# tomtor/HDL-deflate

Measured on AMD Instinct MI355X. Metric: compress_input_throughput (CWINDOW=32, MATCH10=True, static tree), higher is better.
Workload: dtype u8; 1 GPU; BASELINE configs[1]: 1048576 x 2048 B blocks, families 1-4 (test_deflate.py:38-66), distinct blocks, HBM-resident; cwindow=32, maxmatch=10, blocks_per_gpu=1048576, block_bytes=2048

## Files before the change

hdl_deflate_amd/csrc/hdlz_compress.hip:

```cpp
#include <hip/hip_runtime.h>
#include <stdint.h>
#include "hdlz_device.h"
#include "hdlz_compress_common.h"

namespace hdlz {

#ifndef HDLZ_HP_SEARCH
#define HDLZ_HP_SEARCH 1
#define HDLZ_HP_EXTEND 0
#define HDLZ_HP_REST 0
#endif
#ifdef HDLZ_TILE_TIMING
#define TT_DECL() uint32_t tacc[13] = {0, 0, 0, 0, 0, 0, 0, 0, 0, 0, 0, 0, 0}, tlast = (uint32_t)__builtin_readcyclecounter(); \
        const uint32_t tt_c0 = tlast, tt_r0 = (uint32_t)__builtin_amdgcn_s_memrealtime()
#define TT(k) do { const uint32_t t_ = (uint32_t)__builtin_readcyclecounter(); tacc[k] += t_ - tlast; tlast = t_; } while (0)
#define TT_TILE() tacc[12] += 1u
#else
#define TT_DECL() do {} while (0)
#define TT(k) do {} while (0)
#define TT_TILE() do {} while (0)
#endif

__device__ __forceinline__ void store_words(uint32_t* __restrict__ dst, const uint32_t* lsrc, uint32_t words, uint32_t lane) {
    const uint32_t nq = words >> 2;
    for (uint32_t q0 = 0; q0 < nq; q0 += 64u) {
        const uint32_t q = q0 + lane;
        if (q < nq) {
            const v4 v = *reinterpret_cast<const v4*>(lsrc + 4u * q);
            asm volatile("global_store_dwordx4 %0, %1, off\n\ts_nop 1" :: "v"(dst + 4u * q), "v"(v) : "memory");
        }
    }
    if (lane < (words & 3u)) dst[4u * nq + lane] = lsrc[4u * nq + lane];
}

template <int NCH, bool FULLWIN, bool ONE_TILE, bool ENDBITS = false>
__global__ __launch_bounds__(64) __attribute__((amdgpu_waves_per_eu(waves_eu<NCH>(), waves_eu<NCH>()))) void k_compress(CompressArgs a) {
    constexpr bool HASH = wide_hash<NCH>();
    constexpr bool BITS = ONE_TILE && NCH == 1 && search_bits();
    __shared__ typename std::conditional<HASH, WaveLdsNoOut, typename std::conditional<BITS, WaveLdsBits, WaveLds>::type>::type lds;
    __shared__ typename std::conditional<HASH, HashLds<NCH>, uint32_t>::type hl;
    uint32_t* const lout = lds_out(lds, hl);
    const uint32_t lane = threadIdx.x;

    if constexpr (!BITS) {
        fill_luts<NCH>(lds.lut, lane);
        __syncthreads();
    }

    const uint32_t cw4 = 4u * (uint32_t)a.cwindow;
    const uint32_t kmax = (uint32_t)a.maxmatch;
    uint8_t* lin8 = reinterpret_cast<uint8_t*>(lds.in);
    const uint8_t* lut8 = reinterpret_cast<const uint8_t*>(lds.lut);
    uint8_t* out8 = reinterpret_cast<uint8_t*>(lout);

    const uint32_t fixed_st = a.in_len < 5u ? (uint32_t)HDLZ_E_SHORT_INPUT
                            : (ONE_TILE && a.in_len > (uint32_t)TILE) ? (uint32_t)HDLZ_E_BAD_PARAM
                            : (uint64_t)out_bound(a.in_len) > a.out_pitch ? (uint32_t)HDLZ_E_OUT_CAPACITY : (uint32_t)HDLZ_OK;
    auto block_params = [&](uint64_t blk, const uint8_t*& src, uint32_t& n) -> uint32_t {
        if (!a.in_off) {
            src = a.in + blk * a.in_pitch;
            n = a.in_len;
            return fixed_st;
        }
        const uint64_t off = a.in_off[blk];
        const uint64_t len64 = a.in_off[blk + 1] - off;
        if (len64 >= 0x80000000ull) return HDLZ_E_BAD_PARAM;
        n = (uint32_t)len64;
        src = a.in + off;
        if (n < 5u) return HDLZ_E_SHORT_INPUT;
        if (ONE_TILE && n > (uint32_t)TILE) return HDLZ_E_BAD_PARAM;
        if ((uint64_t)out_bound(n) > a.out_pitch) return HDLZ_E_OUT_CAPACITY;
        return HDLZ_OK;
    };
    constexpr uint32_t NCHUNK = (TILE + LOOKAHEAD) / 16;
    const uint32_t in_base = (uint32_t)__builtin_amdgcn_readfirstlane((int)(uint32_t)reinterpret_cast<uintptr_t>(lin8)) + (uint32_t)HALO;
    auto request_tile = [&](const uint8_t* tsrc, uint32_t nfull) {
        if (lane < nfull) lds_dma16(tsrc + 16u * lane, in_base);
        if (lane + 64u < nfull) lds_dma16(tsrc + 16u * (lane + 64u), in_base + 1024u);
        if (nfull > 128u) { if (lane == 0u) lds_dma16(tsrc + 2048u, in_base + 2048u); }
    };
    [[maybe_unused]] const uint32_t lut_base = (uint32_t)__builtin_amdgcn_readfirstlane((int)(uint32_t)reinterpret_cast<uintptr_t>(lds.lut));
    auto request_lut = [&]() {
        const uint8_t* t = reinterpret_cast<const uint8_t*>(FIXED_LUT.e) + 16u * lane;
        lds_dma16(t, lut_base);
        lds_dma16(t + 1024u, lut_base + 1024u);
    };

#if defined(HDLZ_STRIDE_PLAIN) || defined(HDLZ_TILE_TIMING)
    constexpr bool MOVING_COLUMN = false;
#else
    constexpr bool MOVING_COLUMN = BITS;
#endif
    [[maybe_unused]] uint64_t row0 = 0;
    [[maybe_unused]] uint32_t col = blockIdx.x;
    auto next_block = [&](uint64_t& blk) {
        if constexpr (MOVING_COLUMN) {
            row0 += gridDim.x;
            col = col + 1u == gridDim.x ? 0u : col + 1u;
            blk = row0 + col;
        } else blk += gridDim.x;
    };
    TT_DECL();
    for (uint64_t blk = blockIdx.x; blk < a.nblocks; next_block(blk)) {
        const uint8_t* src;
        uint32_t n;
        const uint32_t bst = block_params(blk, src, n);
        if (bst != HDLZ_OK) {
            if (lane == 0) {
                a.out_len[blk] = 0; a.status[blk] = bst;
                if constexpr (ENDBITS) a.end_bits[blk] = 0;
            }
            continue;
        }
        uint32_t* __restrict__ outw = reinterpret_cast<uint32_t*>(a.out + blk * a.out_pitch);
        const uint32_t mis = (uint32_t)(reinterpret_cast<uintptr_t>(src) & 3u);
        const bool aligned16 = (reinterpret_cast<uintptr_t>(src) & 15u) == 0;

        uint32_t gw = 0;
        uint32_t base_bits = HEADER_BITS;
        uint32_t carry_word = HEADER_WORD;
        uint32_t skip_in = 0;
        uint32_t ad_a = 0, ad_w = 0;
        uint32_t wm = (n - min(lane * (uint32_t)RUN, n)) % ADLER_MOD;

        for (uint32_t t0 = 0; t0 < n; t0 += TILE) {
            if (blk == blockIdx.x) TT(10); else TT(0);
            HDLZ_MARK("stage");
            const uint32_t nfull = min((n - t0) >> 4, NCHUNK);
            wave_lds_order();
            lds.in[lane] = t0 != 0 ? lds.in[(TILE / 4) + lane] : 0u;
            asm volatile("s_waitcnt lgkmcnt(0)" ::: "memory");
            request_tile(src + t0, nfull);
            {
                const uint32_t part = (nfull < NCHUNK && ((n - t0) & 15u) != 0u) ? 1u : 0u;
                for (uint32_t c = nfull + part + lane; c < NCHUNK; c += 64) *reinterpret_cast<uint4*>(lin8 + HALO + c * 16u) = make_uint4(0, 0, 0, 0);
                if (part) {
                    if (lane == 0u) *reinterpret_cast<uint4*>(lin8 + HALO + nfull * 16u) = load_chunk16(src, t0 + nfull * 16u, n, aligned16, mis);
                }
            }
            if constexpr (!HASH && !BITS) zero_bit_buffer(lout, lane, carry_word);
            asm volatile("s_waitcnt vmcnt(0)" ::: "memory");
            wave_lds_order();

            const uint32_t run_dw = (HALO / 4) + lane * (RUN / 4);
            const uint32_t p_run = t0 + lane * RUN;
            const uint32_t nrem = n - min(p_run, n);
            uint32_t best[RUN], tok[RUN], code[RUN];
            [[maybe_unused]] uint32_t oww[12];
            [[maybe_unused]] bool any = true;
            [[maybe_unused]] uint32_t planes[7];
            if constexpr (BITS) {
                load_own(lds.in, run_dw, oww);
                asm volatile("s_waitcnt lgkmcnt(0)" ::: "memory");
                wave_lds_order();
            }
            TT(1);
            if constexpr (!HASH) __builtin_amdgcn_s_setprio(0);
            else __builtin_amdgcn_s_setprio(HDLZ_HP_SEARCH);
            HDLZ_MARK("search");
            if constexpr (HASH) {
                match_search_hash<NCH>(lds.in, hl, lane, (uint32_t)a.cwindow, best);
                zero_bit_buffer(lout, lane, carry_word);
            }
#ifndef HDLZ_SEARCH_KEYS
            else if constexpr (BITS)
                any = match_search_bits<true>(oww[0], oww[1], oww[2], oww[3], oww[4], oww[5], oww[6], oww[7], planes, lds.neq + lane, end_cap_word((int32_t)(n - t0) - 2, lane * (uint32_t)RUN));
#endif
            else match_search<NCH, ONE_TILE && NCH == 1>(lds.in, run_dw, best);
            {
                TT(2);
                HDLZ_MARK("adler");
                uint32_t ow[12];
                if constexpr (BITS) {
#pragma unroll
                    for (int k = 0; k < 12; k++) ow[k] = oww[k];
                } else load_own(lds.in, run_dw, ow);
                {
                    uint32_t sa, sc;
                    adler_run(ow, sa, sc);
                    ad_a += sa;
                    ad_w = (ad_w + __umul24(wm, sa) + (4u * ADLER_MOD - sc)) % ADLER_MOD;
                    wm = wm >= (uint32_t)(TILE % ADLER_MOD) ? wm - (uint32_t)(TILE % ADLER_MOD) : wm + (ADLER_MOD - (uint32_t)(TILE % ADLER_MOD));
                    if (((t0 >> 11) & 0x3FFFFu) == 0x3FFFFu) ad_a %= ADLER_MOD;
                    asm volatile("" : "+v"(ad_a), "+v"(ad_w), "+v"(wm));
                }
                TT(3);
                if constexpr (!HASH) __builtin_amdgcn_s_setprio(1);
                else __builtin_amdgcn_s_setprio(HDLZ_HP_EXTEND);
                HDLZ_MARK("extend");
                if constexpr (BITS) {
                    if (any) {
#if HDLZ_EXT_SDWA
                        uint32_t Q[8];
                        search_result_packed(planes, Q);
                        wave_lds_order();
                        make_tokens_bits_packed<FULLWIN>(lds.neq, lane, ow, Q, cw4, kmax, tok, (int32_t)(n - t0));
#else
                        search_result_bytes(planes, best);
                        wave_lds_order();
                        make_tokens_bits<FULLWIN>(lds.neq, lane, ow, best, cw4, kmax, 4u * min(p_run, 32u * NCH), tok, (int32_t)(n - t0));
#endif
                    } else {
                        literal_tokens(ow, tok);
                        asm volatile("s_waitcnt lgkmcnt(0)" ::: "memory");
                        wave_lds_order();
                    }
                } else
                make_tokens<NCH, FULLWIN, true>(lds.in, HALO + lane * RUN, ow, best, cw4, kmax, 4u * min(p_run, 32u * NCH), nrem, tok, (int32_t)(n - t0));
            }
            pin(tok);
            PHASE_FENCE();
            TT(4);
            if constexpr (BITS) {
                HDLZ_MARK("zero");
                wave_lds_order();
                request_lut();
                zero_bit_buffer(lout, lane, carry_word);
            }
            if constexpr (HASH) __builtin_amdgcn_s_setprio(HDLZ_HP_REST);
            HDLZ_MARK("parse");
            uint32_t myskip = 0;
            if (!BITS || any) {
                const uint64_t P = run_transfer(tok);
                TT(5);
                HDLZ_MARK("chain");
                myskip = chain_skips(P, lane, skip_in);
            }
            pin(tok); asm volatile("" : "+v"(myskip));
            PHASE_FENCE();
            TT(6);
            HDLZ_MARK("codes");
            if constexpr (BITS) {
                asm volatile("s_waitcnt vmcnt(0)" ::: "memory");
                wave_lds_order();
            }
            uint32_t lane_bits = token_codes<NCH, false>(lut8, tok, myskip, 0u, code);
            pin(code);
            PHASE_FENCE();
            TT(7);
            HDLZ_MARK("scan");
            uint32_t incl = wave_scan_incl(lane_bits);
            const uint32_t tile_bits_all = (uint32_t)__builtin_amdgcn_readlane((int)incl, 63);
            pin(code); asm volatile("" : "+v"(incl), "+v"(lane_bits));
            PHASE_FENCE();
            TT(8);
            HDLZ_MARK("scatter");
            scatter_codes(out8, code, base_bits + incl - lane_bits);
            TT(9);
            HDLZ_MARK("flush");
            wave_lds_order();
            TT(10);

            const bool last = ONE_TILE || (t0 + TILE >= n);
            if (!last) {
                const uint32_t end_bits = base_bits + tile_bits_all;
                const uint32_t full = end_bits >> 5;
                store_words(outw + gw, lout, full, lane);
                carry_word = lout[full];
                gw += full;
                base_bits = end_bits & 31u;
            } else {
                const uint32_t ninv = t0 + TILE - n;
                const uint32_t end_bits = base_bits + tile_bits_all - PAD_BITS * ninv;
                if (lane < 4u) wipe_behind(lout, end_bits, lane);
                uint32_t s1, s2;
                adler_finish(wave_sum(ad_a % ADLER_MOD), wave_sum(ad_w), n, s1, s2);
                const uint32_t nbytes = block_nbytes(end_bits);
                wave_lds_order();
                if (lane == 0) put_adler(out8, nbytes, s1, s2);
                wave_lds_order();
                const uint32_t total = nbytes + 4u;
                const uint32_t words = (total + 3u) >> 2;
                store_words(outw + gw, lout, words, lane);
                if (lane == 0) {
                    a.out_len[blk] = gw * 4u + total;
                    a.status[blk] = HDLZ_OK;
                    if constexpr (ENDBITS) a.end_bits[blk] = 32ull * gw + end_bits;
                }
            }
            TT(11);
            TT_TILE();
        }
    }
#ifdef HDLZ_TILE_TIMING
    asm volatile("s_waitcnt vmcnt(0)" ::: "memory");
    if (lane == 0) {
        uint64_t blk = blockIdx.x;
#pragma unroll
        for (int k = 0; k < 13; k++, blk += gridDim.x)
            if (blk < a.nblocks) { a.out_len[blk] = tacc[k]; a.status[blk] = 0u; }
        if (blk < a.nblocks) { a.out_len[blk] = (uint32_t)__builtin_readcyclecounter() - tt_c0; a.status[blk] = 0u; }
        blk += gridDim.x;
        if (blk < a.nblocks) { a.out_len[blk] = (uint32_t)__builtin_amdgcn_s_memrealtime() - tt_r0; a.status[blk] = 0u; }
    }
#endif
}

template __global__ void k_compress<1, true, true>(CompressArgs);
template __global__ void k_compress<1, false, true>(CompressArgs);
template __global__ void k_compress<1, true, false>(CompressArgs);
template __global__ void k_compress<1, false, false>(CompressArgs);
template __global__ void k_compress<2, true, false>(CompressArgs);
template __global__ void k_compress<2, false, false>(CompressArgs);
template __global__ void k_compress<8, true, false>(CompressArgs);
template __global__ void k_compress<8, false, false>(CompressArgs);
template __global__ void k_compress<1, true, true, true>(CompressArgs);
template __global__ void k_compress<1, false, true, true>(CompressArgs);
template __global__ void k_compress<1, true, false, true>(CompressArgs);
template __global__ void k_compress<1, false, false, true>(CompressArgs);
template __global__ void k_compress<2, true, false, true>(CompressArgs);
template __global__ void k_compress<2, false, false, true>(CompressArgs);
template __global__ void k_compress<8, true, false, true>(CompressArgs);
template __global__ void k_compress<8, false, false, true>(CompressArgs);

hipError_t launch_compress(const CompressArgs& a, hipStream_t stream) {
    if (a.nblocks == 0) return hipSuccess;
    static int ncu_of[64] = {0};
    int dev = 0;
    if (hipGetDevice(&dev) != hipSuccess) return hipGetLastError();
    int ncu = (dev >= 0 && dev < 64) ? ncu_of[dev] : 0;
    if (ncu == 0) {
        if (hipDeviceGetAttribute(&ncu, hipDeviceAttributeMultiprocessorCount, dev) != hipSuccess) return hipGetLastError();
        if (ncu <= 0) ncu = 256;
        if (dev >= 0 && dev < 64) ncu_of[dev] = ncu;
    }
    if (!a.end_bits && a.in_len >= 5u && a.in_len <= 1024u && a.out_pitch >= (uint64_t)out_bound(a.in_len) &&
        (a.in_off || ((a.in_pitch & 15u) == 0 && (reinterpret_cast<uintptr_t>(a.in) & 15u) == 0)))
        return launch_compress_small(a, stream, ncu);
    uint64_t g = (uint64_t)ncu * 256u;
    if (g > a.nblocks) g = a.nblocks;
    const dim3 grid((unsigned)g), block(64);
    const bool one_tile = a.in_len >= 5u && a.in_len <= (uint32_t)TILE;
    with_window(a.cwindow, [&](auto N, auto FW) {
        constexpr int NCH = decltype(N)::value;
        constexpr bool FULLWIN = decltype(FW)::value;
        if (a.end_bits) {
            if (NCH == 1 && one_tile) hipLaunchKernelGGL((k_compress<1, FULLWIN, true, true>), grid, block, 0, stream, a);
            else hipLaunchKernelGGL((k_compress<NCH, FULLWIN, false, true>), grid, block, 0, stream, a);
        } else if (NCH == 1 && one_tile) hipLaunchKernelGGL((k_compress<1, FULLWIN, true>), grid, block, 0, stream, a);
        else hipLaunchKernelGGL((k_compress<NCH, FULLWIN, false>), grid, block, 0, stream, a);
    });
    return hipGetLastError();
}

}
```

hdl_deflate_amd/csrc/hdlz_compress_common.h:

```cpp
#pragma once
#include <hip/hip_runtime.h>
#include <stddef.h>
#include <stdint.h>
#include "hdlz_device.h"
#include "hdlz_adler.h"

namespace hdlz {

#ifndef HDLZ_W1
#define HDLZ_W1 5
#endif

#ifndef HDLZ_EXT_GROUP
#define HDLZ_EXT_GROUP 4
#endif
#ifndef HDLZ_CODE_GROUP
#define HDLZ_CODE_GROUP 4
#endif
constexpr int RUN = 32;
constexpr int TILE = 64 * RUN;
constexpr int HALO = 256;
constexpr int LOOKAHEAD = 16;
constexpr int IN_BYTES = HALO + TILE + LOOKAHEAD;
constexpr int OUT_WORDS = 592;
// ... 97 lines not shown
    }
    const uint32_t dcode = __builtin_bitreverse32(c) >> 27;
    return (((dcode | (extra << 5)) << 7) << CODE_SHIFT) | ((12u + eb) << NB_SHIFT);
}
__host__ __device__ constexpr uint32_t length_code(uint32_t m) { return (__builtin_bitreverse32(m - 2u) >> 25) << CODE_SHIFT; }
static_assert(literal_entry(0) == (0x0Cu << CODE_SHIFT | 8u << NB_SHIFT), "literal 0: 8 bits, 00110000 reversed");
static_assert(literal_entry(143) == (0xFDu << CODE_SHIFT | 8u << NB_SHIFT), "literal 143: 8 bits, 10111111 reversed");
static_assert(literal_entry(144) == (0x13u << CODE_SHIFT | 9u << NB_SHIFT), "literal 144: 9 bits, 110010000 reversed");
static_assert(literal_entry(255) == (0x1FFu << CODE_SHIFT | 9u << NB_SHIFT), "literal 255: 9 bits, all ones");
static_assert(length_code(3) == 0x40u << CODE_SHIFT && length_code(10) == 0x08u << CODE_SHIFT, "lengths 3 / 10: symbols 257 / 264 = 7-bit codes 0000001 / 0001000 reversed");
static_assert(dist_entry(1) == (12u << NB_SHIFT), "distance 1: code 0, no extra bits: 7 + 5 bits");
static_assert(dist_entry(5) == ((0x04u << 7) << CODE_SHIFT | 13u << NB_SHIFT), "distance 5: code 4 (00100), one extra bit 0");
static_assert(dist_entry(32) == (((0x12u | 7u << 5) << 7) << CODE_SHIFT | 15u << NB_SHIFT), "distance 32: code 9 (01001 reversed), three extra bits 111");
static_assert(dist_entry(256) == (((0x1Eu | 63u << 5) << 7) << CODE_SHIFT | 18u << NB_SHIFT), "distance 256: code 15 (01111 reversed), six extra bits 111111: the widest entry");

__host__ __device__ constexpr uint32_t match_entry32(uint32_t e) { return dist_entry((e & 31u) + 1u) | length_code((e >> 5) + 3u); }
struct __attribute__((aligned(16))) FixedLut { uint32_t e[LUT_LIT + LUT_MATCH]; };
constexpr FixedLut make_fixed_lut() {
    FixedLut t{};
    for (uint32_t k = 0; k < (uint32_t)LUT_LIT; k++) t.e[k] = literal_entry(k);
    for (uint32_t k = 0; k < (uint32_t)LUT_MATCH; k++) t.e[LUT_LIT + k] = match_entry32(k);
    return t;
}
static __device__ const FixedLut FIXED_LUT = make_fixed_lut();
static_assert(make_fixed_lut().e[LUT_LIT + 32 * 7 + 31] == (dist_entry(32) | length_code(10)), "match [len - 3][dist - 1]");


__device__ __forceinline__ void load_own(const uint32_t* in, uint32_t run_dw, uint32_t (&ow)[12]) {
    const uint4 v0 = *reinterpret_cast<const uint4*>(&in[run_dw]);
    const uint4 v1 = *reinterpret_cast<const uint4*>(&in[run_dw + 4]);
    const uint4 v2 = *reinterpret_cast<const uint4*>(&in[run_dw + 8]);
    ow[0] = v0.x; ow[1] = v0.y; ow[2] = v0.z; ow[3] = v0.w;
    ow[4] = v1.x; ow[5] = v1.y; ow[6] = v1.z; ow[7] = v1.w;
    ow[8] = v2.x; ow[9] = v2.y; ow[10] = v2.z; ow[11] = v2.w;
}

constexpr uint32_t NO_MATCH4 = 0x8004u;
template <int NCH, bool PREV_DPP = false>
__device__ __forceinline__ void match_search(const uint32_t* in, uint32_t run_dw, uint32_t (&best)[RUN]) {
    uint32_t ko[RUN];
    uint32_t ow0;
    {
        uint32_t ow[12];
        load_own(in, run_dw, ow);
        static_for<0, RUN>([&](auto I) { constexpr int i = decltype(I)::value; ko[i] = key3<i>(ow, (uint32_t)(4 * (i + 32))); });
        ow0 = ow[0];
    }
    pin(ko); asm volatile("" : "+v"(ow0));
    PHASE_FENCE();
#pragma unroll
    for (int i = 0; i < RUN; i++) best[i] = NCH == 1 ? 0xFFFFFFFFu : NO_MATCH4;

#pragma unroll 1
    for (int k = NCH - 1; k >= 0; k--) {
        uint32_t cd[17];
        const uint32_t cdw = run_dw - 8u * (uint32_t)(k + 1);
        [[maybe_unused]] uint32_t m128 = 0xFFFFFF80u;
        if constexpr (PREV_DPP) {
            static_assert(NCH == 1, "own keys double as the next lane's candidates only for a 32-wide window");
            asm volatile("" : "+v"(m128));
#pragma unroll
            for (int j = 0; j < 17; j++) cd[j] = 0;
        } else {
            const uint4 c0 = *reinterpret_cast<const uint4*>(&in[cdw]);
            const uint4 c1 = *reinterpret_cast<const uint4*>(&in[cdw + 4]);
            cd[0] = c0.x; cd[1] = c0.y; cd[2] = c0.z; cd[3] = c0.w;
            cd[4] = c1.x; cd[5] = c1.y; cd[6] = c1.z; cd[7] = c1.w;
            if (NCH == 1) {
                cd[8] = ow0;
#pragma unroll
                for (int j = 9; j < 17; j++) cd[j] = 0;
            } else {
                const uint4 c2 = *reinterpret_cast<const uint4*>(&in[cdw + 8]);
                const uint4 c3 = *reinterpret_cast<const uint4*>(&in[cdw + 12]);
                cd[8] = c2.x; cd[9] = c2.y; cd[10] = c2.z; cd[11] = c2.w;
                cd[12] = c3.x; cd[13] = c3.y; cd[14] = c3.z; cd[15] = c3.w;
                cd[16] = in[cdw + 16];
            }
        }
        uint32_t m[RUN];
#pragma unroll
        for (int i = 0; i < RUN; i++) m[i] = 0xFFFFFFFFu;
        static_for<0, 63>([&](auto J) {
            constexpr int j = decltype(J)::value;
            if constexpr ((j & 1) == 0) {
                uint32_t kc0, kc1;
                if constexpr (NCH == 1 && j >= 32) {
                    asm volatile("" : "+v"(ko[j - 32]), "+v"(ko[j - 31]));
                    kc0 = ko[j - 32];
                    kc1 = ko[j - 31];
                } else if constexpr (PREV_DPP) {
                    kc0 = (uint32_t)__builtin_amdgcn_update_dpp(0, (int)ko[j], 0x13C, 0xF, 0xF, false) + m128;
                    kc1 = (uint32_t)__builtin_amdgcn_update_dpp(0, (int)ko[j + 1], 0x13C, 0xF, 0xF, false) + m128;
                } else {
                    kc0 = key3<j>(cd, (uint32_t)(4 * j));
                    kc1 = key3<j + 1>(cd, (uint32_t)(4 * (j + 1)));
                }
                static_for<0, RUN>([&](auto I) {
                    constexpr int i = decltype(I)::value;
                    constexpr bool use0 = (j >= i) && (j <= i + 31);
                    constexpr bool use1 = (j + 1 >= i) && (j + 1 <= i + 31);
                    if constexpr (use0 && use1) m[i] = umin3(m[i], ko[i] - kc0, ko[i] - kc1);
                    else if constexpr (use0) m[i] = min(m[i], ko[i] - kc0);
                    else if constexpr (use1) m[i] = min(m[i], ko[i] - kc1);
                });
                if constexpr ((j & 7) == 6) { pin(m); PHASE_FENCE(); }
            }
        });
#pragma unroll
        for (int i = 0; i < RUN; i++) {
            if (NCH == 1) best[i] = m[i];
            else if (m[i] < 256u) best[i] = m[i] + 128u * (uint32_t)k;
        }
    }
}

constexpr uint32_t B3_SEL = 0xE4;
constexpr uint32_t B3_OR_XOR = 0xF6;
constexpr uint32_t B3_OR3 = 0xFE;
constexpr uint32_t B3_OR_ANDN = 0xF4;
template <uint32_t F>
__device__ __forceinline__ uint32_t bitop3(uint32_t a, uint32_t b, uint32_t c) { return __builtin_amdgcn_bitop3_b32(a, b, c, F); }
__device__ __forceinline__ uint32_t sconst(uint32_t v) { asm volatile("" : "+s"(v)); return v; }
__device__ __forceinline__ void exchange8(uint32_t (&w)[8]) {
    static_for<0, 3>([&](auto J) {
        constexpr int s = 1 << decltype(J)::value;
        const uint32_t m0 = sconst(s == 1 ? 0x55555555u : s == 2 ? 0x33333333u : 0x0F0F0F0Fu);
#pragma unroll
        for (int k = 0; k < 8; k++) {
            if (k & s) continue;
            const uint32_t x = w[k], y = w[k + s];
            w[k] = bitop3<B3_SEL>(x, y << s, m0);
            w[k + s] = bitop3<B3_SEL>(x >> s, y, m0);
        }
    });
}
__device__ __forceinline__ void transpose4x4_bytes(uint32_t r0, uint32_t r1, uint32_t r2, uint32_t r3, uint32_t& t0, uint32_t& t1,
                                                   uint32_t& t2, uint32_t& t3) {
    const uint32_t zip_lo = sconst(0x05010400u), zip_hi = sconst(0x07030602u), cat_lo = sconst(0x05040100u), cat_hi = sconst(0x07060302u);
    const uint32_t a01 = __builtin_amdgcn_perm(r1, r0, zip_lo), b01 = __builtin_amdgcn_perm(r1, r0, zip_hi);
    const uint32_t a23 = __builtin_amdgcn_perm(r3, r2, zip_lo), b23 = __builtin_amdgcn_perm(r3, r2, zip_hi);
    t0 = __builtin_amdgcn_perm(a23, a01, cat_lo); t1 = __builtin_amdgcn_perm(a23, a01, cat_hi);
    t2 = __builtin_amdgcn_perm(b23, b01, cat_lo); t3 = __builtin_amdgcn_perm(b23, b01, cat_hi);
}
constexpr bool skip_dead_planes() {
#ifdef HDLZ_PLANES_ALL_LIVE
    return false;
#else
    return true;
#endif
}
constexpr bool literal_tiles() {
#ifdef HDLZ_NO_LITERAL_TILE
    return false;
#else
    return true;
#endif
}
__device__ __forceinline__ uint32_t end_cap_word(int32_t n_m2, uint32_t p_run) {
    const int32_t first = min(max(n_m2 - (int32_t)p_run, 0), 32);
    return (uint32_t)(~0ull << first);
}
template <bool KEEP>
__device__ __forceinline__ bool match_search_bits(uint32_t x0, uint32_t x1, uint32_t x2, uint32_t x3, uint32_t x4, uint32_t x5, uint32_t x6,
                                                  uint32_t x7, uint32_t (&R)[7], [[maybe_unused]] uint32_t* neq_col = nullptr, uint32_t E = 0u) {
    uint32_t O[8];
    transpose4x4_bytes(x0, x2, x4, x6, O[0], O[1], O[2], O[3]);
    transpose4x4_bytes(x1, x3, x5, x7, O[4], O[5], O[6], O[7]);
    exchange8(O);
    pin(O);
    PHASE_FENCE();
    uint32_t nq[RUN];
    static_for<0, 8>([&](auto B) {
        constexpr int b = decltype(B)::value;
        bool live = true;
        if constexpr (b != 0 && skip_dead_planes()) {
            const uint32_t s0 = (uint32_t)__builtin_amdgcn_readfirstlane((int)O[b]);
            live = !((s0 == 0u || s0 == 0xFFFFFFFFu) && ballot64(O[b] != s0) == 0ull);
        }
        if (live) {
            const uint32_t Pb = (uint32_t)__builtin_amdgcn_mov_dpp((int)O[b], 0x13C, 0xF, 0xF, false);
            static_for<1, RUN + 1>([&](auto Dd) {
                constexpr int d = decltype(Dd)::value;
                const uint32_t c = d == 32 ? Pb : __builtin_amdgcn_alignbit(O[b], Pb, (uint32_t)(32 - d));
                if constexpr (b == 0) nq[d - 1] = bitop3<B3_OR_XOR>(E, O[0], c);
                else nq[d - 1] = bitop3<B3_OR_XOR>(nq[d - 1], O[b], c);
                if constexpr ((d & 3) == 0) { pin_range<d - 4, d>(nq); PHASE_FENCE(); }
            });
        }
        pin(nq);
        PHASE_FENCE();
    });
    uint32_t G = 0xFFFFFFFFu, D[6] = {0, 0, 0, 0, 0, 0};
    static_for<1, RUN + 1>([&](auto Dd) {
        constexpr int d = decltype(Dd)::value;
        const uint32_t neq = nq[d - 1];
        if constexpr (KEEP) neq_col[(d & (NEQ_ROWS - 1)) * 64] = neq;
        const uint32_t nx = (uint32_t)__builtin_amdgcn_mov_dpp((int)neq, 0x130, 0xF, 0xF, true);
        const uint32_t n3 = bitop3<B3_OR3>(neq, __builtin_amdgcn_alignbit(nx, neq, 1u), __builtin_amdgcn_alignbit(nx, neq, 2u));
        static_for<0, 6>([&](auto K) {
            constexpr int k = decltype(K)::value;
            if constexpr ((d >> k) & 1) D[k] = bitop3<B3_OR_ANDN>(D[k], G, n3);
        });
        G &= n3;
        if constexpr ((d & 3) == 0) { pin(D); asm volatile("" : "+v"(G)); PHASE_FENCE(); }
    });
    R[0] = G;
#pragma unroll
    for (int k = 0; k < 6; k++) R[k + 1] = D[k];
    if constexpr (literal_tiles()) return ballot64(G != 0xFFFFFFFFu) != 0ull;
    else return true;
}
__device__ __forceinline__ void search_result_packed(const uint32_t (&R)[7], uint32_t (&Q)[8]) {
    const uint32_t G = R[0];
    Q[0] = G; Q[1] = G;
#pragma unroll
    for (int k = 2; k < 8; k++) Q[k] = R[k - 1] | G;
    exchange8(Q);
}
__device__ __forceinline__ void search_result_bytes(const uint32_t (&R)[7], uint32_t (&best)[RUN]) {
    uint32_t Q[8];
    search_result_packed(R, Q);
#pragma unroll
    for (int k = 0; k < 8; k++) {
        best[k] = Q[k] & 0xFFu;
        best[k + 8] = __builtin_amdgcn_ubfe(Q[k], 8u, 8u);
        best[k + 16] = __builtin_amdgcn_ubfe(Q[k], 16u, 8u);
        best[k + 24] = Q[k] >> 24;
    }
}
template <int NCH> struct HashCfg {
#ifndef HDLZ_HASH_BITS
#define HDLZ_HASH_BITS 10
#endif
    static constexpr int HB = HDLZ_HASH_BITS;
    static constexpr int NT = 1 << HB;
    static constexpr int PRE = 64 * ((32 * NCH + 63) / 64);
    static_assert(PRE <= HALO && HB >= 8 && HB <= 16, "halo / tag position");
    static_assert(32 * NCH <= PRE, "cwindow <= PRE: chain walks must stay inside the entries this tile has written (ADVICE r3)");
};
template <int NCH> struct __attribute__((aligned(16))) HashLds {
    union {
        uint32_t T[HashCfg<NCH>::NT];
        uint16_t D[TILE];
    };
    uint16_t E[HALO + TILE];
    static_assert(sizeof(uint32_t) * HashCfg<NCH>::NT >= sizeof(uint16_t) * TILE, "D overlays T");
};

__device__ __forceinline__ uint32_t* lds_out(WaveLds& l, uint32_t&) { return l.out; }
__device__ __forceinline__ uint32_t* lds_out(WaveLdsBits& l, uint32_t&) { return l.out; }
template <int NCH> __device__ __forceinline__ uint32_t* lds_out(WaveLdsNoOut&, HashLds<NCH>& h) {
    static_assert(sizeof(h.T) >= sizeof(uint32_t) * OUT_WORDS, "the bit buffer overlays T / D");
    return h.T;
}

template <int NCH>
__device__ __forceinline__ void match_search_hash(const uint32_t* in, HashLds<NCH>& hl, uint32_t lane, uint32_t cw, uint32_t (&best)[RUN]) {
    constexpr int HB = HashCfg<NCH>::HB, NT = HashCfg<NCH>::NT, PRE = HashCfg<NCH>::PRE;
    constexpr uint32_t base = HALO - PRE;
    for (uint32_t k = lane * 4u; k < (uint32_t)NT; k += 256u) *reinterpret_cast<uint4*>(&hl.T[k]) = make_uint4(0, 0, 0, 0);
    __syncthreads();

    constexpr int G = 8;
    static_assert(RUN % G == 0 && PRE / 64 <= G, "groups");
    uint32_t res2[RUN / 2];
    struct Grp { uint32_t kw[G], ow[G], c0[G], dd[G]; };
    auto hash_of = [&](uint32_t kw, uint32_t& tag) -> uint32_t {
        uint32_t mix;
        asm("v_mul_u32_u24 %0, %1, %2" : "=v"(mix) : "v"(kw), "v"(0x9E3779u));
        tag = (mix << (HB - 8)) & 0xFF00u;
        return __builtin_amdgcn_ubfe(mix, 24 - HB, HB);
    };
    auto issue = [&](auto G0, auto CNT, Grp& q) {
        constexpr int g0 = decltype(G0)::value, cnt = decltype(CNT)::value;
        uint32_t w0_[cnt], w1_[cnt];
        static_for<0, cnt>([&](auto J) {
            constexpr int j = decltype(J)::value;
            const uint32_t idx = base + 64u * (uint32_t)(g0 + j) + lane;
            w0_[j] = in[idx >> 2]; w1_[j] = in[(idx >> 2) + 1u];
        });
        static_for<0, cnt>([&](auto J) {
            constexpr int j = decltype(J)::value;
            constexpr uint32_t rbase = base + 64u * (uint32_t)(g0 + j);
            q.kw[j] = alignbyte(w1_[j], w0_[j], lane);
            const uint32_t h = hash_of(q.kw[j], q.ow[j]);
            q.c0[j] = __hip_atomic_fetch_max(&hl.T[h], rbase + lane, __ATOMIC_RELAXED, __HIP_MEMORY_SCOPE_WORKGROUP);
        });
    };
    auto reorder = [&](uint32_t rbase, uint32_t kw, uint32_t got) -> uint32_t {
        uint32_t tag;
        const uint32_t h = hash_of(kw, tag);
        uint32_t before = got, nearer = 0u;
        bool has = false;
#pragma unroll 1
        for (uint32_t s_ = 0; s_ < 64u; s_++) {
            const uint32_t hs = (uint32_t)__builtin_amdgcn_readlane((int)h, (int)s_), gs = (uint32_t)__builtin_amdgcn_readlane((int)got, (int)s_);
            if (hs == h) {
                before = min(before, gs);
                if (s_ < lane) { nearer = rbase + s_; has = true; }
            }
        }
        return has ? nearer : before;
    };
    auto consume = [&](auto G0, auto CNT, Grp& q) {
        constexpr int g0 = decltype(G0)::value, cnt = decltype(CNT)::value;
        uint32_t inv = 0;
        static_for<0, cnt>([&](auto J) {
            constexpr int j = decltype(J)::value;
            inv |= (base + 64u * (uint32_t)(g0 + j) + lane) - q.c0[j];
        });
#ifdef HDLZ_HASH_FORCE_REORDER
        inv = 0x80000000u;
#endif
        if (ballot64((int32_t)inv < 0) != 0ull) {
            static_for<0, cnt>([&](auto J) {
                constexpr int j = decltype(J)::value;
                q.c0[j] = reorder(base + 64u * (uint32_t)(g0 + j), q.kw[j], q.c0[j]);
            });
        }
        static_for<0, cnt>([&](auto J) {
            constexpr int j = decltype(J)::value;
            constexpr uint32_t rbase = base + 64u * (uint32_t)(g0 + j);
            const uint32_t idx = rbase + lane;
            const uint32_t d = idx - q.c0[j];
            hl.E[idx] = (uint16_t)(q.ow[j] | min(d - 1u, 255u));
            q.dd[j] = (d - 1u) < cw ? d : 0u;
        });
    };
    auto walk = [&](auto G0, Grp& q) {
        constexpr int g0 = decltype(G0)::value;
        uint32_t ev_[G], found_[G];
        auto step = [&](uint32_t ev, uint32_t ow, uint32_t& dd, uint32_t& found) {
            const uint32_t nd = dd + (ev & 255u) + 1u;
            const bool live = dd != 0u;
            const bool same = (ev ^ ow) < 256u;
            found = (live & same) ? dd : found;
            dd = (live & !same & (nd <= cw)) ? nd : 0u;
        };
#pragma unroll
        for (int pass = 0; pass < 2; pass++) {
            static_for<0, G>([&](auto J) {
                constexpr int j = decltype(J)::value;
                ev_[j] = hl.E[base + 64u * (uint32_t)(g0 + j) + lane - q.dd[j]];
            });
            static_for<0, G>([&](auto J) {
                constexpr int j = decltype(J)::value;
                if (pass == 0) found_[j] = 0u;
                step(ev_[j], q.ow[j], q.dd[j], found_[j]);
            });
        }
        static_for<0, G>([&](auto J) {
            constexpr int j = decltype(J)::value;
            const uint32_t idx = base + 64u * (uint32_t)(g0 + j) + lane;
            while (ballot64(q.dd[j] != 0u) != 0ull) step(hl.E[idx - q.dd[j]], q.ow[j], q.dd[j], found_[j]);
        });
        uint32_t c0_[G], c1_[G];
        static_for<0, G>([&](auto J) {
// ... 195 lines not shown
    const uint8_t* neq8 = reinterpret_cast<const uint8_t*>(neq);
    const uint32_t col_lo = 4u * lane, dcol = min(252u - col_lo, 4u);
    const uint32_t tok_k = sconst((2u << 18) + LUT_MATCH_BYTE - 4u), row_mask = sconst(0x7Cu), two = sconst(2u), cw4v = cw4;
    uint32_t T = lane == 0u ? 0x60402000u : 0xE0C0A080u;
    asm volatile("" : "+v"(T));
    static_for<0, RUN>([&](auto J) {
        constexpr int k = decltype(J)::value >> 2, m = decltype(J)::value & 3, i = k + 8 * m;
        if constexpr (m == 0 && k != 0) T += 0x04040404u;
        uint64_t okm = le_byte<m, true>(Q[k], T);
        if constexpr (!FULLWIN) okm &= le_byte<m, false>(Q[k], cw4v);
        okm &= ((uint32_t)i <= thr ? m_hi : m_lo);
        uint32_t a0;
        asm("v_lshl_add_u32 %0, %1, 6, %2" : "=v"(a0) : "v"(and_byte<m>(Q[k], row_mask)), "v"(col_lo));
        uint32_t x;
        if constexpr (i + 3 + 7 <= 32) x = *reinterpret_cast<const uint32_t*>(neq8 + a0) >> (i + 3);
        else if constexpr (i + 3 >= 32) x = *reinterpret_cast<const uint32_t*>(neq8 + (a0 + dcol)) >> (i + 3 - 32);
        else x = __builtin_amdgcn_alignbit(*reinterpret_cast<const uint32_t*>(neq8 + (a0 + dcol)), *reinterpret_cast<const uint32_t*>(neq8 + a0), (uint32_t)(i + 3));
        uint32_t z;
        asm("v_ffbl_b32 %0, %1" : "=v"(z) : "v"(x));
        const uint32_t l3 = min(z, kmax_m3);
        const uint32_t lit = shl_byte<(i & 3)>(two, ow[i >> 2]);
        uint32_t mt;
        asm("v_mad_u32_u24 %0, %1, %2, %3" : "=v"(mt) : "v"(l3), "s"(tok_mul), "v"(add_byte<m>(Q[k], tok_k)));
        asm("v_cndmask_b32_e64 %0, %1, %2, %3" : "=v"(tok[i]) : "v"(lit), "v"(mt), "s"(okm));
        if constexpr (m == 3) { asm volatile("" : "+v"(tok[k]), "+v"(tok[k + 8]), "+v"(tok[k + 16]), "+v"(tok[k + 24]), "+v"(T)); PHASE_FENCE(); }
    });
}
template <bool FULLWIN>
__device__ __forceinline__ void make_tokens_bits(const uint32_t* neq, uint32_t lane, uint32_t (&ow)[12], uint32_t (&best)[RUN], uint32_t cw4,
                                                 uint32_t kmax, uint32_t p4_run, uint32_t (&tok)[RUN], int32_t tile_rem) {
    pin(best); pin_range<0, 8>(ow);
    PHASE_FENCE();
    const uint32_t kmax_m3 = min(kmax - 3u, 7u);
    const int32_t rem5 = tile_rem - 5;
    const uint32_t thr = rem5 >= 0 ? ((uint32_t)rem5 & 31u) : 0u;
    const int32_t cnt_hi = rem5 >= 0 ? (rem5 >> 5) + 1 : 0, cnt_lo = rem5 >= 0 ? (rem5 >> 5) : 0;
    const uint64_t m_hi = cnt_hi >= 64 ? ~0ull : ((1ull << cnt_hi) - 1ull), m_lo = cnt_lo >= 64 ? ~0ull : ((1ull << cnt_lo) - 1ull);
    const uint32_t tok_k = (2u << 18) + LUT_MATCH_BYTE - 4u;
    const uint32_t tok_mul = 4u * 65536u + 128u;
    const uint8_t* neq8 = reinterpret_cast<const uint8_t*>(neq);
    const uint32_t col_lo = 4u * lane, dcol = 4u * min(lane + 1u, 63u) - col_lo;
    static_for<0, RUN>([&](auto I) {
        constexpr int i = decltype(I)::value;
        const uint32_t d4 = best[i];
        uint64_t okm = __builtin_amdgcn_ballot_w64(d4 <= p4_run + (uint32_t)(4 * i));
        if constexpr (!FULLWIN) okm &= __builtin_amdgcn_ballot_w64(d4 <= cw4);
        okm &= ((uint32_t)i <= thr ? m_hi : m_lo);
        uint32_t a0;
        asm("v_lshl_add_u32 %0, %1, 6, %2" : "=v"(a0) : "v"(d4 & 0x7Cu), "v"(col_lo));
        uint32_t x;
        if constexpr (i + 3 + 7 <= 32) x = *reinterpret_cast<const uint32_t*>(neq8 + a0) >> (i + 3);
        else if constexpr (i + 3 >= 32) x = *reinterpret_cast<const uint32_t*>(neq8 + (a0 + dcol)) >> (i + 3 - 32);
        else x = __builtin_amdgcn_alignbit(*reinterpret_cast<const uint32_t*>(neq8 + (a0 + dcol)), *reinterpret_cast<const uint32_t*>(neq8 + a0), (uint32_t)(i + 3));
        uint32_t z;
        asm("v_ffbl_b32 %0, %1" : "=v"(z) : "v"(x));
        const uint32_t l3 = min(z, kmax_m3);
        const uint32_t lit = literal_token<i>(ow);
        uint32_t mt;
        asm("v_mad_u32_u24 %0, %1, %2, %3" : "=v"(mt) : "v"(l3), "s"(tok_mul), "v"(d4 + tok_k));
        asm("v_cndmask_b32_e64 %0, %1, %2, %3" : "=v"(tok[i]) : "v"(lit), "v"(mt), "s"(okm));
        constexpr int EG = HDLZ_EXT_GROUP;
        if constexpr ((i & (EG - 1)) == EG - 1) { pin_range<(i & ~(EG - 1)), (i & ~(EG - 1)) + EG>(tok); PHASE_FENCE(); }
    });
}

__device__ __forceinline__ uint64_t run_transfer(const uint32_t (&tok)[RUN]) {
    uint64_t P = 0x9876543210ull;
#pragma unroll
    for (int i = RUN - 1; i >= 0; i--) {
        const uint32_t sh = tok[i] >> 16;
        const uint32_t e = (uint32_t)(P >> sh) & 15u;
        P = (P << 4) | e;
    }
    return P;
}

constexpr int CHAIN_STEPS = 4;
__device__ __forceinline__ uint32_t chain_skips_serial(uint64_t P, uint32_t lane, uint32_t& s);
__device__ __forceinline__ uint32_t chain_skips(uint64_t P, uint32_t lane, uint32_t& s) {
    const uint32_t plo = (uint32_t)P, phi = (uint32_t)(P >> 32) & 0xFFu;
#ifndef HDLZ_CHAIN_SERIAL_ONLY
    const uint32_t dl = plo ^ __builtin_amdgcn_alignbit(phi, plo, 4u), dh = (phi ^ (phi >> 4)) & 15u;
    uint32_t x = (dl | dh) == 0u ? (plo & 15u) : 16u;
#ifdef HDLZ_CHAIN_FORCE_SERIAL
    x = 16u;
#endif
    bool open = ballot64(x >= 16u) != 0ull;
#pragma unroll 1
    for (int it = 0; it < CHAIN_STEPS && open; it++) {
        const uint32_t prev = (uint32_t)__builtin_amdgcn_update_dpp((int)s, (int)x, 0x138, 0xF, 0xF, false);
        const uint32_t via = (uint32_t)(P >> (4u * (prev & 15u))) & 15u;
        x = (x >= 16u && prev < 16u) ? via : x;
        open = ballot64(x >= 16u) != 0ull;
    }
    if (!open) {
        const uint32_t e = (uint32_t)__builtin_amdgcn_update_dpp((int)s, (int)x, 0x138, 0xF, 0xF, false);
        s = (uint32_t)__builtin_amdgcn_readlane((int)x, 63);
        return e;
    }
#endif
    return chain_skips_serial(P, lane, s);
}
__device__ __forceinline__ uint32_t chain_skips_serial(uint64_t P, uint32_t lane, uint32_t& s) {
    const uint32_t plo = (uint32_t)P;
    uint32_t ph4 = (uint32_t)(P >> 32) & 0xFFu;
    ph4 |= (uint32_t)__builtin_amdgcn_mov_dpp((int)ph4, 0xB1, 0xF, 0xF, true) << 8;
    ph4 |= (uint32_t)__builtin_amdgcn_mov_dpp((int)ph4, 0x4E, 0xF, 0xF, true) << 16;
    uint64_t sv[4] = {0, 0, 0, 0};
    static_for<0, 4>([&](auto G) {
        constexpr int g = decltype(G)::value;
        uint64_t acc = 0;
#pragma unroll
        for (int q = 0; q < 4; q++) {
            const uint32_t hi4 = (uint32_t)__builtin_amdgcn_readlane((int)ph4, g * 16 + q * 4);
#pragma unroll
            for (int k = 0; k < 4; k++) {
                const int l = q * 4 + k;
                acc |= (uint64_t)s << (4 * l);
                const uint64_t f = ((uint64_t)((hi4 >> (8 * k)) & 0xFFu) << 32) |
                                   (uint64_t)(uint32_t)__builtin_amdgcn_readlane((int)plo, g * 16 + l);
                s = (uint32_t)(f >> (4u * s)) & 15u;
            }
        }
        sv[g] = acc;
        __builtin_amdgcn_sched_barrier(0);
    });
    const uint32_t g = lane >> 4;
    const uint64_t mine = g == 0 ? sv[0] : g == 1 ? sv[1] : g == 2 ? sv[2] : sv[3];
    return (uint32_t)(mine >> (4u * (lane & 15u))) & 15u;
}

template <int NCH, bool LIMIT>
__device__ __forceinline__ uint32_t token_codes(const uint8_t* lut8, uint32_t (&tok)[RUN], uint32_t c0, uint32_t nlimit,
                                                uint32_t (&code)[RUN]) {
    uint32_t acc = 0;
    uint32_t c = 4u * c0;
    static_for<0, RUN>([&](auto I) {
        constexpr int i = decltype(I)::value;
        const uint32_t e = *reinterpret_cast<const uint32_t*>(lut8 + (tok[i] & 0xFFFFu));
        bool start = (c == 0u);
        if constexpr (LIMIT) start = start & ((uint32_t)i < nlimit);
        const uint32_t lenm1x4 = tok[i] >> 16;
        c = start ? lenm1x4 : (c - 4u);
        uint32_t ee = e;
        if constexpr (NCH != 1)
            ee |= *reinterpret_cast<const uint32_t*>(lut8 + LUT_LEN_BYTE + lenm1x4);
        code[i] = start ? ee : 0u;
        acc += code[i];
        constexpr int CG = HDLZ_CODE_GROUP;
        if constexpr ((i & (CG - 1)) == CG - 1) { pin_range<(i & ~(CG - 1)), (i & ~(CG - 1)) + CG>(code); asm volatile("" : "+v"(c), "+v"(acc)); PHASE_FENCE(); }
    });
    return (acc & NB_SUM_MASK) >> NB_SHIFT;
}

__device__ __forceinline__ uint32_t wave_scan_incl(uint32_t v) {
    v += (uint32_t)__builtin_amdgcn_update_dpp(0, (int)v, 0x111, 0xF, 0xF, true);
    v += (uint32_t)__builtin_amdgcn_update_dpp(0, (int)v, 0x112, 0xF, 0xF, true);
    v += (uint32_t)__builtin_amdgcn_update_dpp(0, (int)v, 0x114, 0xF, 0xF, true);
    v += (uint32_t)__builtin_amdgcn_update_dpp(0, (int)v, 0x118, 0xF, 0xF, true);
    v += (uint32_t)__builtin_amdgcn_update_dpp(0, (int)v, 0x142, 0xA, 0xF, false);
    v += (uint32_t)__builtin_amdgcn_update_dpp(0, (int)v, 0x143, 0xC, 0xF, false);
    return v;
}

__device__ __forceinline__ void scatter_codes(uint8_t* out8, const uint32_t (&code)[RUN], uint32_t bp) {
#pragma unroll
    for (int i = 0; i < RUN; i += 2) {
        const uint32_t n0 = (code[i] & NB_MASK) >> NB_SHIFT;
        const uint32_t c = ((code[i + 1] >> CODE_SHIFT) << n0) | (code[i] >> CODE_SHIFT);
        const uint64_t v = (uint64_t)c << (bp & 31u);
        uint32_t* w = reinterpret_cast<uint32_t*>(out8 + ((bp >> 3) & ~3u));
        __hip_atomic_fetch_or(w, (uint32_t)v, __ATOMIC_RELAXED, __HIP_MEMORY_SCOPE_WORKGROUP);
        __hip_atomic_fetch_or(w + 1, (uint32_t)(v >> 32), __ATOMIC_RELAXED, __HIP_MEMORY_SCOPE_WORKGROUP);
        bp += n0 + ((code[i + 1] & NB_MASK) >> NB_SHIFT);
        if ((i & 6) == 6) { asm volatile("" : "+v"(bp)); PHASE_FENCE(); }
    }
}

__device__ __forceinline__ void adler_run(const uint32_t (&ow)[12], uint32_t& sa, uint32_t& sc) {
    sa = 0; sc = 0;
#pragma unroll
    for (int k = 0; k < 8; k++) {
        sa = __builtin_amdgcn_sad_u8(ow[k], 0u, sa);
        const uint32_t wts = (uint32_t)(4 * k) | ((uint32_t)(4 * k + 1) << 8) | ((uint32_t)(4 * k + 2) << 16) | ((uint32_t)(4 * k + 3) << 24);
        sc = __builtin_amdgcn_udot4(ow[k], wts, sc, false);
    }
}

__device__ __forceinline__ uint32_t wave_sum(uint32_t v) {
    v += (uint32_t)__builtin_amdgcn_update_dpp(0, (int)v, 0xB1, 0xF, 0xF, true);
    v += (uint32_t)__builtin_amdgcn_update_dpp(0, (int)v, 0x4E, 0xF, 0xF, true);
    v += (uint32_t)__builtin_amdgcn_update_dpp(0, (int)v, 0x141, 0xF, 0xF, true);
    v += (uint32_t)__builtin_amdgcn_update_dpp(0, (int)v, 0x140, 0xF, 0xF, true);
    return (uint32_t)__builtin_amdgcn_readlane((int)v, 0) + (uint32_t)__builtin_amdgcn_readlane((int)v, 16) +
           (uint32_t)__builtin_amdgcn_readlane((int)v, 32) + (uint32_t)__builtin_amdgcn_readlane((int)v, 48);
}

constexpr uint32_t HEADER_WORD = 0x78u | (0x9Cu << 8) | (0x3u << 16);
constexpr uint32_t HEADER_BITS = 19;
constexpr uint32_t PAD_BITS = 8;
__device__ __forceinline__ void wipe_behind(uint32_t* lout, uint32_t end_bits, uint32_t k) {
    const uint32_t ew = end_bits >> 5, rb = end_bits & 31u;
    lout[ew + k] = (k == 0u) ? (lout[ew] & ((1u << rb) - 1u)) : 0u;
}
template <class U> __device__ __forceinline__ U block_nbytes(U end_bits) { return (end_bits + 7u + 7u) >> 3; }
__device__ __forceinline__ uint32_t member_len(uint32_t n, uint64_t E, uint64_t pitch, uint32_t& body) {
    body = 0u;
    if (E < HEADER_BITS || block_nbytes(E) + 4u != (uint64_t)n || (uint64_t)n > pitch) return 0u;
    const uint32_t nbytes = n - 4u;
    const uint32_t p = (uint32_t)(8ull * nbytes - E) - 7u;
    body = nbytes - 2u;
    return body + (p >= 3u ? 4u : 5u);
}
template <class U> __device__ __forceinline__ void adler_finish(U A, U W, uint32_t n, uint32_t& s1, uint32_t& s2) {
    s1 = (uint32_t)((A + 1u) % ADLER_MOD);
    s2 = (uint32_t)((W + n % ADLER_MOD) % ADLER_MOD);
}
__device__ __forceinline__ uint32_t adler_byte(uint32_t k, uint32_t s1, uint32_t s2) {
    const uint32_t s = k < 2u ? s2 : s1;
    return (k & 1u) ? (s & 255u) : (s >> 8);
}
__device__ __forceinline__ void put_adler(uint8_t* out8, uint32_t nbytes, uint32_t s1, uint32_t s2) {
#pragma unroll
    for (uint32_t k = 0; k < 4u; k++) out8[nbytes + k] = (uint8_t)adler_byte(k, s1, s2);
}

__device__ __forceinline__ void zero_bit_buffer(uint32_t* lout, uint32_t lane, uint32_t carry_word) {
    static_assert(OUT_WORDS % 4 == 0, "16-byte stores");
    for (uint32_t q = lane; q < (uint32_t)OUT_WORDS / 4u; q += 64u)
        *reinterpret_cast<uint4*>(lout + 4u * q) = make_uint4(q == 0u ? carry_word : 0u, 0u, 0u, 0u);
}

template <int NCH>
__device__ __forceinline__ void fill_luts(uint32_t* lut, uint32_t lane) {
    for (uint32_t e = lane; e < (uint32_t)LUT_LIT; e += 64) lut[e] = literal_entry(e);
    for (uint32_t e = lane; e < (uint32_t)LUT_MATCH; e += 64) {
        if (NCH == 1) lut[LUT_LIT + e] = match_entry32(e);
        else lut[LUT_LIT + e] = dist_entry(e + 1u);
    }
    if (lane < (uint32_t)LUT_LEN) lut[LUT_LIT + LUT_MATCH + lane] = lane ? length_code(lane + 1u) : 0u;
}

__device__ __forceinline__ void zero_tail16(uint4& v, uint32_t valid) {
    uint32_t* vv = reinterpret_cast<uint32_t*>(&v);
#pragma unroll
    for (int k = 0; k < 4; k++) {
        const uint32_t lo = 4u * k;
        const uint32_t m = valid <= lo ? 0u : (valid >= lo + 4u ? 0xFFFFFFFFu : ((1u << (8u * (valid - lo))) - 1u));
        vv[k] &= m;
    }
}

__device__ __forceinline__ uint4 load_chunk16(const uint8_t* __restrict__ src, uint32_t p, uint32_t n, bool aligned16, uint32_t mis) {
    uint4 v;
    if (aligned16) {
        v = *reinterpret_cast<const uint4*>(src + p);
    } else {
        const uint32_t* q = reinterpret_cast<const uint32_t*>(src + p - mis);
        const uint32_t nd = (n - p + mis + 3u) >> 2;
        uint32_t d0 = q[0];
        uint32_t d1 = nd > 1 ? q[1] : 0, d2 = nd > 2 ? q[2] : 0, d3 = nd > 3 ? q[3] : 0, d4 = nd > 4 ? q[4] : 0;
        v.x = alignbyte(d1, d0, mis);
        v.y = alignbyte(d2, d1, mis);
        v.z = alignbyte(d3, d2, mis);
        v.w = alignbyte(d4, d3, mis);
    }
    const uint32_t valid = n - p;
    if (valid < 16u) zero_tail16(v, valid);
    return v;
}

__device__ __forceinline__ void stage_tile(uint8_t* lin8, const uint8_t* __restrict__ src, uint32_t t0, uint32_t n, bool aligned16,
                                           uint32_t mis, uint32_t lane) {
    __syncthreads();
    const uint32_t nchunk = (HALO + TILE + LOOKAHEAD) / 16;
    for (uint32_t c = lane; c < nchunk; c += 64) {
        const int64_t p = (int64_t)t0 - HALO + (int64_t)c * 16;
        uint4 v = make_uint4(0, 0, 0, 0);
        if (p >= 0 && p < (int64_t)n) v = load_chunk16(src, (uint32_t)p, n, aligned16, mis);
        *reinterpret_cast<uint4*>(lin8 + c * 16u) = v;
    }
}

}
```

Measured before the change: 893,300 MB/s.

## Add literal-only fast emit path, plain Adler sums for one-tile blocks, grouped planes

When the bit-plane search finds no match in a tile, literal codes are now emitted straight from the LUT using the raw input words. This skips token building, run transfer and skip chaining for that tile. For single-tile blocks the Adler accumulators drop the per-tile modulo reductions and use plain 32-bit sums, guarded by a static_assert on the bounds. The distance-plane computation also groups the higher distance bits per four distances, which cuts bitop work in the search. The cost is extra code paths and branch divergence in the kernel.

```diff
diff --git a/hdl_deflate_amd/csrc/hdlz_compress.hip b/hdl_deflate_amd/csrc/hdlz_compress.hip
--- a/hdl_deflate_amd/csrc/hdlz_compress.hip
+++ b/hdl_deflate_amd/csrc/hdlz_compress.hip
@@ -37,6 +37,7 @@
 __global__ __launch_bounds__(64) __attribute__((amdgpu_waves_per_eu(waves_eu<NCH>(), waves_eu<NCH>()))) void k_compress(CompressArgs a) {
     constexpr bool HASH = wide_hash<NCH>();
     constexpr bool BITS = ONE_TILE && NCH == 1 && search_bits();
+    constexpr bool LIT_EMIT = BITS && literal_emit();
     __shared__ typename std::conditional<HASH, WaveLdsNoOut, typename std::conditional<BITS, WaveLdsBits, WaveLds>::type>::type lds;
     __shared__ typename std::conditional<HASH, HashLds<NCH>, uint32_t>::type hl;
     uint32_t* const lout = lds_out(lds, hl);
@@ -120,8 +121,10 @@
         uint32_t base_bits = HEADER_BITS;
         uint32_t carry_word = HEADER_WORD;
         uint32_t skip_in = 0;
+        constexpr bool ADLER_PLAIN = ONE_TILE && adler_plain_one_tile();
         uint32_t ad_a = 0, ad_w = 0;
-        uint32_t wm = (n - min(lane * (uint32_t)RUN, n)) % ADLER_MOD;
+        uint32_t wm = n - min(lane * (uint32_t)RUN, n);
+        if constexpr (!ADLER_PLAIN) wm %= ADLER_MOD;
 
         for (uint32_t t0 = 0; t0 < n; t0 += TILE) {
             if (blk == blockIdx.x) TT(10); else TT(0);
@@ -167,10 +170,10 @@
                 any = match_search_bits<true>(oww[0], oww[1], oww[2], oww[3], oww[4], oww[5], oww[6], oww[7], planes, lds.neq + lane, end_cap_word((int32_t)(n - t0) - 2, lane * (uint32_t)RUN));
 #endif
             else match_search<NCH, ONE_TILE && NCH == 1>(lds.in, run_dw, best);
+            uint32_t ow[12];
             {
                 TT(2);
                 HDLZ_MARK("adler");
-                uint32_t ow[12];
                 if constexpr (BITS) {
 #pragma unroll
                     for (int k = 0; k < 12; k++) ow[k] = oww[k];
@@ -178,18 +181,36 @@
                 {
                     uint32_t sa, sc;
                     adler_run(ow, sa, sc);
+                    if constexpr (ADLER_PLAIN) {
+                        ad_a = sa;
+                        ad_w = __umul24(wm, sa) - sc;
+                        asm volatile("" : "+v"(ad_a), "+v"(ad_w));
+                    } else {
                     ad_a += sa;
                     ad_w = (ad_w + __umul24(wm, sa) + (4u * ADLER_MOD - sc)) % ADLER_MOD;
                     wm = wm >= (uint32_t)(TILE % ADLER_MOD) ? wm - (uint32_t)(TILE % ADLER_MOD) : wm + (ADLER_MOD - (uint32_t)(TILE % ADLER_MOD));
                     if (((t0 >> 11) & 0x3FFFFu) == 0x3FFFFu) ad_a %= ADLER_MOD;
                     asm volatile("" : "+v"(ad_a), "+v"(ad_w), "+v"(wm));
+                    }
                 }
                 TT(3);
                 if constexpr (!HASH) __builtin_amdgcn_s_setprio(1);
                 else __builtin_amdgcn_s_setprio(HDLZ_HP_EXTEND);
+            }
+            uint32_t lane_bits;
+            if (LIT_EMIT && !any) {
+                HDLZ_MARK("litcodes");
+                asm volatile("s_waitcnt lgkmcnt(0)" ::: "memory");
+                wave_lds_order();
+                request_lut();
+                zero_bit_buffer(lout, lane, carry_word);
+                asm volatile("s_waitcnt vmcnt(0)" ::: "memory");
+                wave_lds_order();
+                if constexpr (LIT_EMIT) lane_bits = literal_codes(lut8, oww, code);
+            } else {
                 HDLZ_MARK("extend");
                 if constexpr (BITS) {
-                    if (any) {
+                    if (LIT_EMIT || any) {
 #if HDLZ_EXT_SDWA
                         uint32_t Q[8];
                         search_result_packed(planes, Q);
@@ -207,34 +228,34 @@
                     }
                 } else
                 make_tokens<NCH, FULLWIN, true>(lds.in, HALO + lane * RUN, ow, best, cw4, kmax, 4u * min(p_run, 32u * NCH), nrem, tok, (int32_t)(n - t0));
-            }
-            pin(tok);
-            PHASE_FENCE();
-            TT(4);
-            if constexpr (BITS) {
-                HDLZ_MARK("zero");
-                wave_lds_order();
-                request_lut();
-                zero_bit_buffer(lout, lane, carry_word);
-            }
-            if constexpr (HASH) __builtin_amdgcn_s_setprio(HDLZ_HP_REST);
-            HDLZ_MARK("parse");
-            uint32_t myskip = 0;
-            if (!BITS || any) {
-                const uint64_t P = run_transfer(tok);
-                TT(5);
-                HDLZ_MARK("chain");
-                myskip = chain_skips(P, lane, skip_in);
-            }
-            pin(tok); asm volatile("" : "+v"(myskip));
-            PHASE_FENCE();
-            TT(6);
-            HDLZ_MARK("codes");
-            if constexpr (BITS) {
-                asm volatile("s_waitcnt vmcnt(0)" ::: "memory");
-                wave_lds_order();
-            }
-            uint32_t lane_bits = token_codes<NCH, false>(lut8, tok, myskip, 0u, code);
+                pin(tok);
+                PHASE_FENCE();
+                TT(4);
+                if constexpr (BITS) {
+                    HDLZ_MARK("zero");
+                    wave_lds_order();
+                    request_lut();
+                    zero_bit_buffer(lout, lane, carry_word);
+                }
+                if constexpr (HASH) __builtin_amdgcn_s_setprio(HDLZ_HP_REST);
+                HDLZ_MARK("parse");
+                uint32_t myskip = 0;
+                if (!BITS || LIT_EMIT || any) {
+                    const uint64_t P = run_transfer(tok);
+                    TT(5);
+                    HDLZ_MARK("chain");
+                    myskip = chain_skips(P, lane, skip_in);
+                }
+                pin(tok); asm volatile("" : "+v"(myskip));
+                PHASE_FENCE();
+                TT(6);
+                HDLZ_MARK("codes");
+                if constexpr (BITS) {
+                    asm volatile("s_waitcnt vmcnt(0)" ::: "memory");
+                    wave_lds_order();
+                }
+                lane_bits = token_codes<NCH, false>(lut8, tok, myskip, 0u, code);
+            }
             pin(code);
             PHASE_FENCE();
             TT(7);
@@ -264,7 +285,8 @@
                 const uint32_t end_bits = base_bits + tile_bits_all - PAD_BITS * ninv;
                 if (lane < 4u) wipe_behind(lout, end_bits, lane);
                 uint32_t s1, s2;
-                adler_finish(wave_sum(ad_a % ADLER_MOD), wave_sum(ad_w), n, s1, s2);
+                if constexpr (ADLER_PLAIN) adler_finish(wave_sum(ad_a), wave_sum(ad_w), n, s1, s2);
+                else adler_finish(wave_sum(ad_a % ADLER_MOD), wave_sum(ad_w), n, s1, s2);
                 const uint32_t nbytes = block_nbytes(end_bits);
                 wave_lds_order();
                 if (lane == 0) put_adler(out8, nbytes, s1, s2);
diff --git a/hdl_deflate_amd/csrc/hdlz_compress_common.h b/hdl_deflate_amd/csrc/hdlz_compress_common.h
--- a/hdl_deflate_amd/csrc/hdlz_compress_common.h
+++ b/hdl_deflate_amd/csrc/hdlz_compress_common.h
@@ -273,6 +273,27 @@
 }
 constexpr bool literal_tiles() {
 #ifdef HDLZ_NO_LITERAL_TILE
+    return false;
+#else
+    return true;
+#endif
+}
+constexpr bool grouped_planes() {
+#ifdef HDLZ_PLANES_PER_DISTANCE
+    return false;
+#else
+    return true;
+#endif
+}
+constexpr bool literal_emit() {
+#ifdef HDLZ_LITERAL_TOKENS
+    return false;
+#else
+    return literal_tiles();
+#endif
+}
+constexpr bool adler_plain_one_tile() {
+#ifdef HDLZ_ADLER_TILE_MOD
     return false;
 #else
     return true;
@@ -313,18 +334,27 @@
         PHASE_FENCE();
     });
     uint32_t G = 0xFFFFFFFFu, D[6] = {0, 0, 0, 0, 0, 0};
+    [[maybe_unused]] uint32_t Gs = 0xFFFFFFFFu;
+    constexpr int KD = grouped_planes() ? 2 : 6;
     static_for<1, RUN + 1>([&](auto Dd) {
         constexpr int d = decltype(Dd)::value;
         const uint32_t neq = nq[d - 1];
         if constexpr (KEEP) neq_col[(d & (NEQ_ROWS - 1)) * 64] = neq;
         const uint32_t nx = (uint32_t)__builtin_amdgcn_mov_dpp((int)neq, 0x130, 0xF, 0xF, true);
         const uint32_t n3 = bitop3<B3_OR3>(neq, __builtin_amdgcn_alignbit(nx, neq, 1u), __builtin_amdgcn_alignbit(nx, neq, 2u));
-        static_for<0, 6>([&](auto K) {
+        static_for<0, KD>([&](auto K) {
             constexpr int k = decltype(K)::value;
             if constexpr ((d >> k) & 1) D[k] = bitop3<B3_OR_ANDN>(D[k], G, n3);
         });
         G &= n3;
-        if constexpr ((d & 3) == 0) { pin(D); asm volatile("" : "+v"(G)); PHASE_FENCE(); }
+        if constexpr (grouped_planes() && ((d & 3) == 3 || d == RUN)) {
+            static_for<2, 6>([&](auto K) {
+                constexpr int k = decltype(K)::value;
+                if constexpr ((d >> k) & 1) D[k] = bitop3<B3_OR_ANDN>(D[k], Gs, G);
+            });
+            Gs = G;
+        }
+        if constexpr ((d & 3) == 0) { pin(D); asm volatile("" : "+v"(G)); if constexpr (grouped_planes()) asm volatile("" : "+v"(Gs)); PHASE_FENCE(); }
     });
     R[0] = G;
 #pragma unroll
@@ -826,6 +856,19 @@
     });
     return (acc & NB_SUM_MASK) >> NB_SHIFT;
 }
+__device__ __forceinline__ uint32_t literal_codes(const uint8_t* lut8, const uint32_t (&ow)[12], uint32_t (&code)[RUN]) {
+    static_assert(4u * 255u + 4u <= 4u * (uint32_t)LUT_LIT, "every byte's offset inside the literal LUT");
+    uint32_t acc = 0;
+    const uint32_t two = sconst(2u);
+    static_for<0, RUN>([&](auto I) {
+        constexpr int i = decltype(I)::value;
+        code[i] = *reinterpret_cast<const uint32_t*>(lut8 + shl_byte<(i & 3)>(two, ow[i >> 2]));
+        acc += code[i];
+        constexpr int CG = HDLZ_CODE_GROUP;
+        if constexpr ((i & (CG - 1)) == CG - 1) { pin_range<(i & ~(CG - 1)), (i & ~(CG - 1)) + CG>(code); asm volatile("" : "+v"(acc)); PHASE_FENCE(); }
+    });
+    return (acc & NB_SUM_MASK) >> NB_SHIFT;
+}
 
 __device__ __forceinline__ uint32_t wave_scan_incl(uint32_t v) {
     v += (uint32_t)__builtin_amdgcn_update_dpp(0, (int)v, 0x111, 0xF, 0xF, true);
@@ -886,6 +929,8 @@
     body = nbytes - 2u;
     return body + (p >= 3u ? 4u : 5u);
 }
+static_assert(64ull * TILE * (RUN * 255ull) < (1ull << 31) && 64ull * (RUN * 255ull) + 1ull < (1ull << 31) && (uint64_t)TILE < (uint64_t)ADLER_MOD,
+              "one-tile blocks: the plain Adler sums of a wave fit 31 bits");
 template <class U> __device__ __forceinline__ void adler_finish(U A, U W, uint32_t n, uint32_t& s1, uint32_t& s2) {
     s1 = (uint32_t)((A + 1u) % ADLER_MOD);
     s2 = (uint32_t)((W + n % ADLER_MOD) % ADLER_MOD);
```

New measurement: 928,200 MB/s, median of 6. +3.9%, better.
